# Aikku93/ulc-codec

Hardware: AMD Instinct MI355X
Metric: encode+decode Msamples/s at BlockSize=2048 stereo (channel-samples through encode+decode, VBR -50, 32 blocks per stream per call) (higher is better)
Workload: dtype f32; 1 GPU; vbr50 (configs[1] encode, configs[2] decode): Batch=4096 independent 44.1 kHz stereo streams/GPU x 32 blocks, BlockSize=2048, VBR -50; step = encode then decode; config=vbr50, mode=both, streams_per_gpu=4096, block_size=2048, channels=2, parallelism=batch split over 1 GPU(s), no collective on the data path

## Files before the change

### ulc-codec_amd/csrc/ulcx_api.cpp

```cpp
#include <math.h>
#include <stddef.h>
#include <stdio.h>
#include <stdlib.h>
#include <string.h>
#include <vector>
#include "ulcx_internal.h"


#define CKR(x) do { hipError_t e_ = (x); if (e_ != hipSuccess) { ulcx_set_error("%s: %s", #x, hipGetErrorString(e_)); return ULCX_ERR_HIP; } } while (0)

struct Block1Graph {
    hipStream_t stream = nullptr; hipGraph_t graph = nullptr; hipGraphExec_t exec = nullptr;
    bool graphed = false, noGraph = false;
};
static void block1_drop(Block1Graph &g) { if (g.graphed) { hipGraphExecDestroy(g.exec); hipGraphDestroy(g.graph); g.graphed = false; } }
template <class F> static int block1_run(Block1Graph &g, F enqueue) {
    if (!g.graphed && !g.noGraph) {
        bool ok = hipStreamBeginCapture(g.stream, hipStreamCaptureModeThreadLocal) == hipSuccess;
        if (ok) {
            const int rc = enqueue();
            hipGraph_t gr = nullptr;
            const hipError_t ee = hipStreamEndCapture(g.stream, &gr);
            ok = (rc == ULCX_OK) && ee == hipSuccess && gr != nullptr;
            if (ok) ok = hipGraphInstantiate(&g.exec, gr, nullptr, nullptr, 0) == hipSuccess;
// ... 112 lines not shown
    for (void *p : e->allocs) hipFree(p);
    if (e->tables) hipFree(e->tables);
    if (e->evOk) for (auto &v : e->ev) hipEventDestroy(v);
    block1_drop(e->b1);
    if (e->b1.stream) hipStreamDestroy(e->b1.stream);
    if (e->pinIn) hipHostFree(e->pinIn);
    if (e->pinOut) hipHostFree(e->pinOut);
    if (e->pinMeta) hipHostFree(e->pinMeta);
    enc_sync_destroy(e->sync);
    delete e;
}

static int enc_reset_state(ulcx_encoder *e) {
    UlcxEncCtx &c = e->ctx;
    CKR(hipMemset(c.hist, 0, sizeof(float) * (size_t)e->B * 2 * e->BS * e->C));
    std::vector<UlcxWcState> w((size_t)e->B);
    for (auto &x : w) {
        memset(&x, 0, sizeof(x));
        x.wcPrev = 0x10;
        x.wcCur  = 0x10;
    }
    CKR(hipMemcpy(c.wcs, w.data(), sizeof(UlcxWcState) * w.size(), hipMemcpyHostToDevice));
    return ULCX_OK;
}

extern "C" int ulcx_encoder_create(ulcx_encoder **out, int device, int nStreams, int nChan, int BlockSize, int RateHz, int maxBlocksPerCall) {
    if (!out) return ULCX_ERR_ARG;
    *out = nullptr;
    if (!validate(nChan, BlockSize) || nStreams < 1 || maxBlocksPerCall < 1 || RateHz < 1) {
        ulcx_set_error("invalid encoder geometry (nStreams=%d nChan=%d BlockSize=%d RateHz=%d maxBlocks=%d)", nStreams, nChan, BlockSize, RateHz, maxBlocksPerCall);
        return ULCX_ERR_ARG;
    }
    if (BlockSize > ULCX_MAX_BS_DEVICE) { ulcx_set_error("BlockSize %d > %d not built for the device yet", BlockSize, ULCX_MAX_BS_DEVICE); return ULCX_ERR_UNSUPPORTED; }
    int rc = select_device(device);
    if (rc) return rc;
    ulcx_encoder *e = new ulcx_encoder();
    e->device = device; e->B = nStreams; e->C = nChan; e->BS = BlockSize; e->rate = RateHz; e->maxK = maxBlocksPerCall;
    UlcxEncCtx &c = e->ctx;
    c.B = nStreams; c.C = nChan; c.BS = BlockSize; c.lgBS = ilog2i(BlockSize); c.maxK = maxBlocksPerCall; c.K = 0;
    c.rateHz = RateHz;
    c.slot = 2 * nChan * BlockSize + 16;
    c.unitCap = 2 * BlockSize + 32;
    c.cHP  = 1.0f - expf(-0x1.CC845Cp6f / RateHz);
    c.cBP  = 1.0f - expf(-0x1.596344p8f / RateHz);
    c.qHP  = 1.0f - expf(-0x1.CC845Cp7f / RateHz);
    c.qBP  = 1.0f - expf(-0x1.596344p8f / RateHz);
    c.cBlk = 1.0f - expf(-0x1.1AF110p-6f * BlockSize / RateHz);
    c.cplxScale = 0x1.62E430p-1f * (31 - __builtin_clz((unsigned)BlockSize));
    rc = ulcx_tables_build(&c.T, &e->tables, BlockSize, RateHz, true);
    if (rc) { cleanup(e); return rc; }
    {
        int most = 0;
        const int N = BlockSize / 2;
        for (int t = 0; t < 2; t++) {
            const short *beg = t ? c.T.pBeg[0] : c.T.nBeg[0], *end = t ? c.T.pEnd[0] : c.T.nEnd[0];
            for (int b = 0; b < ULCX_NBARK; b++) {
                if (beg[b] > end[b] || end[b] > N) most = 1 << 20;
                if (b && (beg[b] < beg[b - 1] || end[b] < end[b - 1])) most = 1 << 20;
            }
            for (int pos = 0; pos <= N; pos++) {
                int open = 0;
                for (int b = 0; b < ULCX_NBARK; b++) open += (beg[b] <= pos && pos <= end[b]) ? 1 : 0;
                if (open > most) most = open;
            }
        }
        int ring = 4;
        while (ring < most) ring *= 2;
        c.barkRing = (ring <= 8 && N % 32 == 0) ? ring : 0;
    }
    size_t B = nStreams, K = maxBlocksPerCall, NB = B * K, cb = (size_t)nChan * BlockSize;
    DA(c.hist, B * 2 * BlockSize * nChan, true);
    DA(c.wcs, B, true);
    DA(c.env, ((B + 63) / 64) * 64 * K * BlockSize, true);
    DA(c.bins, B * (K + 1) * 16, true);
    DA(c.wcArr, B * (K + 2), true);
    DA(c.coef, NB * cb, false);
    DA(c.key, NB * cb, false);
    DA(c.nsum, ((NB * nChan + 63) / 64) * 64 * (size_t)(BlockSize / 2), false);
    DA(c.amp2, ((NB + 63) / 64) * 64 * (size_t)(BlockSize / 2), false);
    DA(c.barkN, NB * nChan * 4 * ULCX_NBARK, true);
    DA(c.barkP, NB * 4 * ULCX_NBARK, true);
    if (c.barkRing) { DA(c.barkRawN, NB * nChan * ULCX_NBARK * 3, false); DA(c.barkRawP, NB * ULCX_NBARK * 3, false); DA(c.decList, NB, false); DA(c.decCount, 1, true); }
    DA(c.nnz, NB, true);
    DA(c.cplx, NB, true);
    DA(c.nout, NB, true);
    DA(c.slow, 3 * NB + 2, true);
    c.useWave = 1;
    c.useGapSums = (cb <= 16384 && nChan <= 16) ? 1 : 0;
    DA(c.gapSum, NB * cb, false);
    DA(c.tailSum, NB * nChan * 4 * 8, true);
    c.directPack = 1;
    if (const char *ev = getenv("ULCX_DIRECT_PACK")) c.directPack = (ev[0] != '0');
    c.dbgSkip = 0;
#ifdef ULCX_ABLATE
    if (const char *ev = getenv("ULCX_DBG_SKIP")) c.dbgSkip = atoi(ev);
#endif
    DA(c.cbrLo, NB, true); DA(c.cbrHi, NB, true); DA(c.cbrDone, NB, true); DA(c.cbrBudget, NB, true); DA(c.cbrLive, 1, true);
    DA(c.selWin, NB, true); DA(c.selT, NB, true); c.selPass = 0;
    { const char *ev = getenv("ULCX_SEL_PAIR"); c.selPair = ev ? atoi(ev) : 1; }
    DA(c.keep, NB * cb / 32, true);
    DA(c.fbList, NB, true);
    DA(c.fbCount, 4, true);
    DA(c.unitBuf, NB * nChan * (size_t)c.unitCap, true);
    DA(c.unitNyb, NB * nChan * 4, true);
    {
        size_t heapBytes = (cb * 8 > ULCX_HEAP_LDS_BYTES) ? (size_t)ULCX_HEAP_GRID * cb * 8 : 16;
        uint8_t *hp = nullptr;
        DA(hp, heapBytes, false);
        c.heapScratch = hp;
    }
    for (auto &v : e->ev) { if (hipEventCreate(&v) != hipSuccess) { ulcx_set_error("hipEventCreate failed"); cleanup(e); return ULCX_ERR_HIP; } }
    e->evOk = true;
    {
        const char *evs = getenv("ULCX_ASYNC_FB");
        const bool sideOk = !(evs && evs[0] == '0') && enc_sync_create(e->sync);
        e->wcPipe = sideOk ? 4 : 1;
        if (const char *pv = getenv("ULCX_WC_PIPE")) { int n = atoi(pv); if (n >= 1 && n <= ULCX_XF_MAXCH && n != 2 && (n == 1 || sideOk)) e->wcPipe = n; }
        if (const char *sv = getenv("ULCX_WC_STEPS")) e->wcSteps = atoi(sv);
    }
    if (const char *av = getenv("ULCX_ANALYSE_KXF")) e->analyseKxf = (av[0] == '1');
    e->nsSlots = c.useGapSums ? ulcx_enc_nsums_slots(BlockSize, nChan) : 0;
    if (e->nsSlots <= 0) e->nsSlots = 1024;
    DA(c.isFb, NB, true);
    DA(c.ownSlot, NB, true);
    {
        size_t slots = NB;
        size_t maxSlots = ((size_t)8 << 30) / (cb * 4);
        size_t freeB = 0, totalB = 0;
        if (hipMemGetInfo(&freeB, &totalB) == hipSuccess && freeB / 4 / (cb * 4) < maxSlots) maxSlots = freeB / 4 / (cb * 4);
        if (maxSlots < 64) maxSlots = 64;
        if (slots > maxSlots) slots = maxSlots;
        if (const char *ev = getenv("ULCX_RANK_SLOTS")) { long n = atol(ev); if (n >= 1 && (size_t)n < slots) slots = (size_t)n; }
        for (;;) {
            int rc_ = dalloc(e->allocs, &c.rankBuf, slots * cb, false);
            if (rc_ == ULCX_OK) break;
            if (rc_ != ULCX_ERR_NOMEM || slots <= 64) { cleanup(e); return rc_; }
            (void)hipGetLastError();
            slots = (slots + 1) / 2; if (slots < 64) slots = 64;
        }
        c.rankSlots = (int)slots;
    }
    rc = enc_reset_state(e);
    if (rc) { cleanup(e); return rc; }
    *out = e;
    return ULCX_OK;
}

extern "C" void ulcx_encoder_destroy(ulcx_encoder *e) { if (e) { hipSetDevice(e->device); cleanup(e); } }
extern "C" int ulcx_encoder_reset(ulcx_encoder *e) { if (!e) return ULCX_ERR_ARG; CKR(hipSetDevice(e->device)); return enc_reset_state(e); }
extern "C" int ulcx_encoder_slot_bytes(const ulcx_encoder *e) { return e ? e->ctx.slot : 0; }

static UlcxEncAux enc_aux(ulcx_encoder *e, int nBlocks) {
    const int wcPipe = (nBlocks >= 2 * e->wcPipe) ? e->wcPipe : (nBlocks >= 6 && e->wcPipe > 1 ? 3 : 1);
    return UlcxEncAux{ e->sync, wcPipe, e->wcSteps, e->wcFuse, e->nsSlots, e->nXf };
}

static int encode_dev_any(ulcx_encoder *e, int mode, float p0, float p1, const ulcx_rate *d_rate, const float *d_pcm, const int16_t *d_pcm16, int nBlocks,
                          uint8_t *d_out, int32_t *d_bits, int32_t *d_wc, float *d_cplx, void *hipStream) {
    if (!e || (!d_pcm && !d_pcm16) || !d_out || !d_bits || nBlocks < 1 || nBlocks > e->maxK) { ulcx_set_error("ulcx_encode_dev: bad argument"); return ULCX_ERR_ARG; }
    if (d_rate) { mode = ULCX_MODE_VBR; p0 = 100.0f; p1 = 0.0f; }
    if (mode != ULCX_MODE_VBR && mode != ULCX_MODE_CBR && mode != ULCX_MODE_ABR) { ulcx_set_error("bad mode"); return ULCX_ERR_ARG; }
    CKR(hipSetDevice(e->device));
    UlcxEncCtx c = e->ctx;
    c.K = nBlocks; c.keyFinal = 0; c.mode = mode; c.p0 = p0; c.p1 = p1;
    c.vbrTarget = (mode == ULCX_MODE_VBR) ? 0x1.E4EFB7p3f * logf(100.0f / p0) : 0.0f;
    c.rates = (const float2 *)d_rate;
// ... 533 lines not shown
extern "C" int ulcx_ulc_rate_kbps(uint64_t totalBytes, uint32_t RateHz, uint32_t BlockSize, uint32_t nBlocks) {
    double avg = (double)totalBytes * 8.0 * RateHz / 1000.0 / ((double)BlockSize * nBlocks);
    return (int)lrint(avg);
}
extern "C" int ulcx_pack_streams_dev(int device, int nStreams, int nBlocks, int slotBytes, const uint8_t *d_slots, const int32_t *d_bits,
                                     uint8_t *d_payload, long long payloadStride, int32_t *d_payloadBytes, int32_t *d_maxBlock, void *hipStream) {
    if (nStreams < 1 || nBlocks < 1 || slotBytes < 1 || !d_slots || !d_bits || !d_payload || !d_payloadBytes || payloadStride < 1) { ulcx_set_error("ulcx_pack_streams_dev: bad argument"); return ULCX_ERR_ARG; }
    int rc = select_device(device);
    if (rc) return rc;
    return ulcx_pack_launch(nStreams, nBlocks, slotBytes, d_slots, d_bits, d_payload, payloadStride, d_payloadBytes, d_maxBlock, (hipStream_t)hipStream);
}
extern "C" int ulcx_decode_packed_dev(ulcx_decoder *e, const uint8_t *d_payload, long long payloadStride, const int32_t *d_payloadBytes,
                                      int nBlocks, float *d_pcm, int32_t *d_bits, void *hipStream) {
    if (!e || !d_payload || !d_payloadBytes || !d_pcm || !d_bits || payloadStride < 1 || nBlocks < 1 || nBlocks > e->maxK) { ulcx_set_error("ulcx_decode_packed_dev: bad argument"); return ULCX_ERR_ARG; }
    CKR(hipSetDevice(e->device));
    UlcxDecCtx c = e->ctx;
    c.K = nBlocks; c.slot = 0; c.in = d_payload; c.pcm = d_pcm; c.pcm16 = nullptr; c.bits = d_bits;
    c.packed = 1; c.payStride = payloadStride; c.payBytes = d_payloadBytes;
    c.inBytes = (long long)e->B * payloadStride;
    int rc = dec_launch(e, c, (hipStream_t)hipStream);
    e->evRecorded = (rc == ULCX_OK) && e->timing;
    return rc;
}
extern "C" int ulcx_decode_packed_host(ulcx_decoder *e, const uint8_t *h_payload, long long payloadStride, const int32_t *h_payloadBytes,
                                       int nBlocks, float *h_pcm, int32_t *h_bits) {
    if (!e || !h_payload || !h_payloadBytes || !h_pcm || !h_bits || nBlocks < 1 || nBlocks > e->maxK || payloadStride < 1) return ULCX_ERR_ARG;
    CKR(hipSetDevice(e->device));
    size_t cb = (size_t)e->C * e->BS, NB = (size_t)e->B * nBlocks;
    uint8_t *dp = nullptr; int32_t *dn = nullptr; float *dpcm = nullptr; int32_t *dbits = nullptr;
    size_t payBytes = (size_t)e->B * (size_t)payloadStride + 16;
    CKR(hipMalloc((void **)&dp, payBytes)); CKR(hipMalloc((void **)&dn, sizeof(int32_t) * e->B));
    CKR(hipMalloc((void **)&dpcm, sizeof(float) * NB * cb)); CKR(hipMalloc((void **)&dbits, sizeof(int32_t) * NB));
    CKR(hipMemset(dp, 0, payBytes));
    CKR(hipMemcpy(dp, h_payload, (size_t)e->B * (size_t)payloadStride, hipMemcpyHostToDevice));
    CKR(hipMemcpy(dn, h_payloadBytes, sizeof(int32_t) * e->B, hipMemcpyHostToDevice));
    int rc = ulcx_decode_packed_dev(e, dp, payloadStride, dn, nBlocks, dpcm, dbits, nullptr);
    if (rc == ULCX_OK) {
        CKR(hipDeviceSynchronize());
        CKR(hipMemcpy(h_pcm, dpcm, sizeof(float) * NB * cb, hipMemcpyDeviceToHost));
        CKR(hipMemcpy(h_bits, dbits, sizeof(int32_t) * NB, hipMemcpyDeviceToHost));
    }
    hipFree(dp); hipFree(dn); hipFree(dpcm); hipFree(dbits);
    return rc;
}

extern "C" int ulcx_decoder_upload_payload(ulcx_decoder *e, const uint8_t *h_payload, long long payloadStride, const int32_t *h_payloadBytes) {
    if (!e || !h_payload || !h_payloadBytes || payloadStride < 1) return ULCX_ERR_ARG;
    CKR(hipSetDevice(e->device));
    if (e->d_pay) { hipFree(e->d_pay); e->d_pay = nullptr; }
    if (e->d_payBytes) { hipFree(e->d_payBytes); e->d_payBytes = nullptr; }
    size_t bytes = (size_t)e->B * (size_t)payloadStride;
    CKR(hipMalloc((void **)&e->d_pay, bytes + 16)); CKR(hipMalloc((void **)&e->d_payBytes, sizeof(int32_t) * e->B));
    CKR(hipMemset(e->d_pay, 0, bytes + 16));
    CKR(hipMemcpy(e->d_pay, h_payload, bytes, hipMemcpyHostToDevice));
    CKR(hipMemcpy(e->d_payBytes, h_payloadBytes, sizeof(int32_t) * e->B, hipMemcpyHostToDevice));
    e->payStride = payloadStride;
    return ulcx_decoder_reset(e);
}
extern "C" int ulcx_decode_resident_host(ulcx_decoder *e, int nBlocks, float *h_pcm, int32_t *h_bits) {
    if (!e || !h_pcm || !h_bits || nBlocks < 1 || nBlocks > e->maxK) return ULCX_ERR_ARG;
    if (!e->d_pay) { ulcx_set_error("ulcx_decode_resident_host: no payload uploaded"); return ULCX_ERR_ARG; }
    CKR(hipSetDevice(e->device));
    size_t cb = (size_t)e->C * e->BS, NB = (size_t)e->B * nBlocks;
    { int rc0 = dec_host_staging(e, (size_t)e->B * e->maxK, 0); if (rc0) return rc0; }
    int rc = ulcx_decode_packed_dev(e, e->d_pay, e->payStride, e->d_payBytes, nBlocks, e->d_pcm, e->d_bits, nullptr);
    if (rc != ULCX_OK) return rc;
    CKR(hipDeviceSynchronize());
    CKR(hipMemcpy(h_pcm, e->d_pcm, sizeof(float) * NB * cb, hipMemcpyDeviceToHost));
    CKR(hipMemcpy(h_bits, e->d_bits, sizeof(int32_t) * NB, hipMemcpyDeviceToHost));
    return ULCX_OK;
}

#ifdef ULCX_DSYN_STAMPS
extern "C" int ulcx_decoder_debug_scratch(ulcx_decoder *e, void *h_out, size_t strideBytes, size_t nBytes, int nStreams);
extern "C" int ulcx_decoder_debug_scratch(ulcx_decoder *e, void *h_out, size_t strideBytes, size_t nBytes, int nStreams) {
    if (!e || !h_out) return ULCX_ERR_ARG;
    CKR(hipSetDevice(e->device));
    CKR(hipDeviceSynchronize());
    for (int s = 0; s < nStreams && s < e->B; s++)
        CKR(hipMemcpy((char *)h_out + (size_t)s * nBytes, (const char *)e->ctx.scratch + (size_t)s * strideBytes, nBytes, hipMemcpyDeviceToHost));
    return ULCX_OK;
}
#endif
extern "C" int ulcx_encoder_set_timing(ulcx_encoder *e, int on) { if (!e) return ULCX_ERR_ARG; e->timing = on != 0; if (!on) e->evRecorded = false; return ULCX_OK; }
extern "C" int ulcx_decoder_set_timing(ulcx_decoder *e, int on) { if (!e) return ULCX_ERR_ARG; e->timing = on != 0; if (!on) e->evRecorded = false; return ULCX_OK; }
static const char *kDecStage[ULCX_DEC_STAGES] = { "k_dscan", "k_dsyn" };
extern "C" const char *ulcx_decoder_stage_name(int i) { return (i >= 0 && i < ULCX_DEC_STAGES) ? kDecStage[i] : ""; }
extern "C" int ulcx_decoder_stage_ms(ulcx_decoder *e, float *ms, int maxStages) {
    if (!e || !e->evRecorded) return 0;
    int n = 0;
    for (int i = 0; i < ULCX_DEC_STAGES && i < maxStages; i++) {
        float t = 0;
        if (hipEventElapsedTime(&t, e->ev[i], e->ev[i + 1]) != hipSuccess) break;
        ms[n++] = t;
    }
    return n;
}
```

### ulc-codec_amd/csrc/ulcx_enc_xf.hip

```cpp
#include "ulcx_enc_dev.h"

__device__ __forceinline__ int first_overlap(int wc, int BS) {
    unsigned p = ulcx_pattern(wc);
    int ov = BS >> (p & 7);
    if (p & 8) ov >>= (wc & 7);
    return ov;
}

__device__ __forceinline__ float win_apply(float x, int i, int S, int aL, int ovL, int aR, int ov,
                                           const float *__restrict__ rise, const float *__restrict__ fall) {
    if (i < S) return (i < aL) ? 0.0f : (i < aL + ovL) ? x * rise[i - aL] : x;
    int n = i - S;
    return (n < aR) ? x : (n < aR + ov) ? x * fall[n - aR] : 0.0f;
}

template <typename IN, int BSC, bool AN = false>
__device__ __forceinline__ int xf_fast(const UlcxEncCtx &c, float *lds, int s, int k, int blk, int tid) {
    constexpr int BS = BSC, S = BSC, M = BSC / 2, PS = 4, Mp = FFT_PADDEDS(M, PS);
    constexpr int LGM = BSC == 4096 ? 11 : 10;
    static_assert(BSC == 2048 || BSC == 4096, "sizes with a compile-time transform");
    static_assert(WG == 256 && (M / 2) % (2 * WG) == 0, "whole fold / epilogue trips per thread");
    float2 *z = (float2 *)lds;
    float2 *twl = (float2 *)(lds + (AN ? 2 : 4) * FFT_PADDEDS(BS, PS));
    float2 *zc0 = z, *zs0 = z + Mp, *zc1 = z + (AN ? 1 : 2) * Mp, *zs1 = z + 3 * Mp;
// ... 70 lines not shown
#pragma unroll
                    for (int p = 0; p < 2; p++) {
                        const int slot = p ? (1 - u) : u;
                        re[q][p][2 * slot] = mdct[2*p] * norm; re[q][p][2 * slot + 1] = mdct[2*p+1] * norm;
                    }
                }
            }
            const int j1 = kA, j2 = M - 1 - kB;
#pragma unroll
            for (int q = 0; q < 2; q++) {
                stnt((float4 *)(coefO + q * BS + 2 * j1), make_float4(re[q][0][0], re[q][0][1], re[q][0][2], re[q][0][3]));
                stnt((float4 *)(coefO + q * BS + 2 * j2), make_float4(re[q][1][0], re[q][1][1], re[q][1][2], re[q][1][3]));
            }
        }
        return 0;
    }
#pragma unroll
    for (int e0 = 0; e0 < M / 2; e0 += 2 * WG) {
        const int kA = e0 + 2 * tid, kB = e0 + 2 * tid + 1;
        const int kk2[2] = { kA, kB };
        float re[2][2][4];
        float ns[2][2][2];
        float am[2][2] = { { 0.0f, 0.0f }, { 0.0f, 0.0f } };
#pragma unroll
        for (int u = 0; u < 2; u++) {
            const int k1 = kk2[u], k2 = M - 1 - k1;
            const int r1 = (int)(__brev((unsigned)k1) >> (32 - LGM)), r2 = (int)(__brev((unsigned)k2) >> (32 - LGM));
            const float2 P1 = pre[k1], P2 = pre[k2];
            const fft_v2f Pv1 = { P1.x, P1.y }, Pv2 = { P2.x, P2.y };
#pragma unroll
            for (int q = 0; q < 2; q++) {
                const float2 *zc = q ? zc1 : zc0, *zs = q ? zs1 : zs0;
                auto cm = [](float2 d, fft_v2f w) { const fft_v2f dv = { d.x, d.y }; const fft_v2f r = fft_cmulc_post_pk(dv, w); return make_float2(r.x, r.y); };
                const float2 yc1 = cm(zc[FFT_PADS(r1, PS)], Pv1), yc2 = cm(zc[FFT_PADS(r2, PS)], Pv2);
                const float2 ys1 = cm(zs[FFT_PADS(r1, PS)], Pv1), ys2 = cm(zs[FFT_PADS(r2, PS)], Pv2);
                const float mdct[4] = { yc1.x, yc2.y, yc2.x, yc1.y };
                const float mdst[4] = { ys1.x, ys2.y, ys2.x, ys1.y };
#pragma unroll
                for (int p = 0; p < 2; p++) {
                    const float re0 = mdct[2*p] * norm,   im0 = mdst[2*p] * norm;
                    const float re1 = mdct[2*p+1] * norm, im1 = mdst[2*p+1] * norm;
                    const float re0s = re0 * re0, im0s = im0 * im0, re1s = re1 * re1, im1s = im1 * im1;
                    const float a0 = re0s + im0s, a1 = re1s + im1s;
                    nnz += (fabsf(re0) < 0.5f * ULCX_COEF_EPS) ? 0 : 1;
                    nnz += (fabsf(re1) < 0.5f * ULCX_COEF_EPS) ? 0 : 1;
                    const int slot = p ? (1 - u) : u;
                    re[q][p][2 * slot] = re0; re[q][p][2 * slot + 1] = re1;
                    ns[q][p][slot] = a0 + a1;
                    am[p][slot] += a0; am[p][slot] += a1;
                }
            }
        }
        const int j1 = kA, j2 = M - 1 - kB;
#pragma unroll
        for (int q = 0; q < 2; q++) {
            stnt((float4 *)(coefO + q * BS + 2 * j1), make_float4(re[q][0][0], re[q][0][1], re[q][0][2], re[q][0][3]));
            stnt((float4 *)(coefO + q * BS + 2 * j2), make_float4(re[q][1][0], re[q][1][1], re[q][1][2], re[q][1][3]));
            stnt((float2 *)(c.nsum + tile_idx(BS / 2, blk * 2 + q, j1)), make_float2(ns[q][0][0], ns[q][0][1]));
            stnt((float2 *)(c.nsum + tile_idx(BS / 2, blk * 2 + q, j2)), make_float2(ns[q][1][0], ns[q][1][1]));
        }
        *(float2 *)(c.amp2 + tile_idx(BS / 2, blk, j1)) = make_float2(am[0][0], am[0][1]);
        *(float2 *)(c.amp2 + tile_idx(BS / 2, blk, j2)) = make_float2(am[1][0], am[1][1]);
    }
    return nnz;
}

template <typename IN>
__device__ __forceinline__ bool xf_is_fast(const UlcxEncCtx &c, int s, int k) {
#ifdef XF_NO_FAST
    return false;
#endif
    const int BS = c.BS;
    const int *wrow = c.wcArr + (size_t)s * (c.maxK + 2) + k;
    const int wcPrev = wrow[0], wc = wrow[1], wcNext = wrow[2];
    if (!(k >= 2 || std::is_same<IN, float>::value) || (ulcx_pattern(wc) >> 4) != 0) return false;
    unsigned pp = ulcx_pattern(wcPrev);
    int lastS = BS;
    do { lastS = BS >> (pp & 7); } while (pp >>= 4);
    int ovFirst = first_overlap(wc, BS);
    if (ovFirst > lastS) ovFirst = lastS;
    return ovFirst == BS && first_overlap(wcNext, BS) >= BS;
}

template <bool ST, typename IN, bool AN = false>
__device__ __forceinline__ void xf_block(const UlcxEncCtx &c, float *lds, int s, int k, const int tid) {
    const int BS = c.BS, C = ST ? 2 : c.C;
    const int blk = s * c.K + k;
    const int ps = ulcx_xf_pad_shift(BS, C);
    float2 *z    = (float2 *)lds;
    constexpr int NA = AN ? 2 : 4;
    float2 *twl  = (float2 *)(lds + NA * FFT_PADDEDS(BS, ps));
    int    &s_nnz = *(int *)(lds + NA * FFT_PADDEDS(BS, ps) + BS / 2);
    const bool ampLds = !AN && (C > 2);
    const bool twInLds = !(ampLds && (size_t)16 * (BS + (BS >> ps)) + (size_t)BS * 4 + 32 > ULCX_LDS_LIMIT);
    float  *amp2 = twInLds ? lds + 4 * FFT_PADDEDS(BS, ps) + BS / 2 + 4 : lds + 4 * FFT_PADDEDS(BS, ps);
    if (!AN && tid == 0) s_nnz = 0;
    if (ampLds) for (int i = tid; i < BS / 2; i += WG) amp2[i] = 0.0f;

    const int *wrow = c.wcArr + (size_t)s * (c.maxK + 2) + k;
    int wcPrev = wrow[0], wc = wrow[1], wcNext = wrow[2];
    if (!AN && c.barkRing && tid == 0 && (ulcx_pattern(wc) & ~8u) != 0) c.decList[atomicAdd(c.decCount, 1)] = blk;
    int nextOv = first_overlap(wcNext, BS);
    int ovFirst;
    {
        unsigned pp = ulcx_pattern(wcPrev);
        int lastS = BS;
        do { lastS = BS >> (pp & 7); } while (pp >>= 4);
        ovFirst = first_overlap(wc, BS);
        if (ovFirst > lastS) ovFirst = lastS;
    }
    size_t cb = (size_t)C * BS;
    float *coefO = c.coef + (size_t)blk * cb;
    int nnz = 0;
    __syncthreads();

#ifdef XF_NO_FAST
    const bool fastBlk = false;
#else
    const bool fastBlk = ST && (BS == 2048 || BS == 4096) && (k >= 2 || std::is_same<IN, float>::value) && (ulcx_pattern(wc) >> 4) == 0
                         && ovFirst == BS && nextOv >= BS;
#endif
    if (fastBlk) nnz = (BS == 2048) ? xf_fast<IN, 2048, AN>(c, lds, s, k, blk, tid) : xf_fast<IN, 4096, AN>(c, lds, s, k, blk, tid);
    else
    for (int ch0 = 0; ch0 < C; ch0 += 2) {
        const int nch = ST ? 2 : ((ch0 + 1 < C) ? 2 : 1);
        unsigned pat = ulcx_pattern(wc);
        int off = 0, ovL = ovFirst;
        do {
            int S = BS >> (pat & 7);
            int d = pat & 7;
            pat >>= 4;
            int ov;
            if (pat) { ov = BS >> (pat & 7); if (pat & 8) ov >>= (wc & 7); }
            else ov = nextOv;
            if (ov > S) ov = S;
            const int M = S >> 1;
            int t0 = (k - 1) * BS - BS / 2 + off - S / 2;
            int aL = (S - ovL) >> 1, aR = (S - ov) >> 1;
            const float *rise = c.T.winRise + ovL, *fall = c.T.winFall + ov;
            const float2 *pre = c.T.pre[d];
            const int Mp = FFT_PADDEDS(M, ps);
            float2 *zc0 = z, *zs0 = z + Mp, *zc1 = z + (AN ? 1 : 2) * Mp, *zs1 = z + 3 * Mp;

            if (twInLds) for (int i = tid; i < M / 2; i += WG) twl[i] = c.T.tw[d][i];
            auto fold = [&](auto inpcmT, auto fullovT) {
                constexpr bool INPCM = decltype(inpcmT)::value, FULLOV = decltype(fullovT)::value;
                const IN *frame = pcm_base<IN>(c) + ((size_t)s * c.K * BS + (INPCM ? t0 : 0)) * C;
                auto ldE = [&](int pos, int e) -> float { return INPCM ? ld1(frame + (size_t)pos * C + e) : smp_ld1<IN>(c, s, t0 + pos, e); };
                auto ldQ = [&](int pos) -> float4 { return INPCM ? ld4(frame + (size_t)pos * C) : smp_ld4<IN>(c, s, t0 + pos); };
                for (int jj = tid; jj < M / 2; jj += WG) {
                    const int iA = 2 * jj, iB = S - 2 - 2 * jj, iC = S + 2 * jj, iD = 2 * S - 2 - 2 * jj;
                    float2 xs[8];
                    {
                        const int ip[4] = { iA, iB, iC, iD };
#pragma unroll
                        for (int r = 0; r < 4; r++) {
                            float2 e0, e1;
                            if (nch == 2) {
                                if (C == 2) { float4 v = ldQ(ip[r]); e0 = make_float2(v.x, v.y); e1 = make_float2(v.z, v.w); }
                                else { e0 = make_float2(ldE(ip[r], ch0), ldE(ip[r], ch0 + 1)); e1 = make_float2(ldE(ip[r] + 1, ch0), ldE(ip[r] + 1, ch0 + 1)); }
                                xs[2 * r]     = make_float2((e0.x + e0.y) * 0.5f, (e0.x - e0.y) * 0.5f);
                                xs[2 * r + 1] = make_float2((e1.x + e1.y) * 0.5f, (e1.x - e1.y) * 0.5f);
                            } else {
                                xs[2 * r] = make_float2(ldE(ip[r], ch0), 0.0f); xs[2 * r + 1] = make_float2(ldE(ip[r] + 1, ch0), 0.0f);
                            }
                        }
                    }
                    const int ipos[8] = { iA, iA + 1, iB, iB + 1, iC, iC + 1, iD, iD + 1 };
#pragma unroll
                    for (int r = 0; r < 8; r++) {
                        if (FULLOV) {
                            float f = (r < 4) ? rise[ipos[r]] : fall[ipos[r] - S];
                            xs[r].x *= f; xs[r].y *= f;
                            continue;
                        }
                        float f; bool zero;
                        if (r < 4) {
                            int idx = ipos[r] - aL;
                            int ci = idx < 0 ? 0 : (idx < ovL ? idx : 0);
                            float tv = rise[ci];
                            f = (idx < ovL) ? tv : 1.0f; zero = idx < 0;
                        } else {
                            int idx = ipos[r] - S - aR;
                            int ci = idx < 0 ? 0 : (idx < ov ? idx : 0);
                            float tv = fall[ci];
                            f = (idx < 0) ? 1.0f : tv; zero = idx >= ov;
                        }
                        float wx = xs[r].x * f, wy = xs[r].y * f;
                        xs[r].x = zero ? 0.0f : wx;
                        xs[r].y = zero ? 0.0f : wy;
                    }
#pragma unroll
                    for (int hsel = 0; hsel < 2; hsel++) {
                        const int n = hsel ? M / 2 + jj : M / 2 - 1 - jj;
                        const float2 lbv = hsel ? xs[0] : xs[1], lav = hsel ? xs[3] : xs[2];
                        const float2 rav = hsel ? xs[4] : xs[5], rbv = hsel ? xs[7] : xs[6];
                        float2 P = pre[n];
#pragma unroll
                        for (int q = 0; q < 2; q++) {
                            if (q >= nch) break;
                            float ra = q ? rav.y : rav.x, rb = q ? rbv.y : rbv.x, la = q ? lav.y : lav.x, lb = q ? lbv.y : lbv.x;
                            float vr = ra + rb, wr = ra - rb;
                            float vl = la - lb, wl = lb + la;
                            float v1 = hsel ? vl : vr, v2 = hsel ? vr : vl;
                            float w1 = hsel ? wl : wr, w2 = hsel ? wr : wl;
                            float2 *zc = q ? zc1 : zc0, *zs = q ? zs1 : zs0;
                            zc[FFT_PADS(n, ps)] = cmulc(make_float2(v1, v2), P);
                            if constexpr (!AN) zs[FFT_PADS(n, ps)] = cmulc(make_float2(w2, w1), P);
                        }
                    }
                }
            };
            if (!(ULCX_DBG(c) & 2)) {
                const bool inPcm = (t0 >= 0), fullOv = (ovL == S) && (ov == S);
                if (inPcm && fullOv) fold(std::true_type{}, std::true_type{});
                else if (inPcm) fold(std::true_type{}, std::false_type{});
                else fold(std::false_type{}, std::false_type{});
            }
            __syncthreads();

            if (!(ULCX_DBG(c) & 1)) for (int a = __builtin_amdgcn_readfirstlane(tid >> 6); a < (AN ? 1 : 2) * nch; a += WG / 64) {
                if (twInLds) fft_wave_dif(z + a * Mp, M, twl, tid & 63, ps);
                else fft_wave_dif(z + a * Mp, M, c.T.tw[d], tid & 63, ps);
            }
            __syncthreads();

            int bits = 31 - __clz(M);
            float norm = 2.0f / S;
            if (!(ULCX_DBG(c) & 4)) for (int kk = tid; kk < M / 2; kk += WG) {
                int k1 = kk, k2 = M - 1 - kk;
                int r1 = (int)(__brev((unsigned)k1) >> (32 - bits));
                int r2 = (int)(__brev((unsigned)k2) >> (32 - bits));
                float2 P1 = pre[k1], P2 = pre[k2];
                float am1 = 0.0f, am2 = 0.0f;
                if (ampLds) { am1 = amp2[off / 2 + k1]; am2 = amp2[off / 2 + k2]; }
#pragma unroll
                for (int q = 0; q < 2; q++) {
                    if (q >= nch) break;
                    int ch = ch0 + q;
                    float2 *zc = q ? zc1 : zc0, *zs = q ? zs1 : zs0;
                    const fft_v2f Pv1 = { P1.x, P1.y }, Pv2 = { P2.x, P2.y };
                    auto cm = [](float2 d, fft_v2f w) { const fft_v2f dv = { d.x, d.y }; const fft_v2f r = fft_cmulc_post_pk(dv, w); return make_float2(r.x, r.y); };
                    float2 yc1 = cm(zc[FFT_PADS(r1, ps)], Pv1), yc2 = cm(zc[FFT_PADS(r2, ps)], Pv2);
                    if constexpr (AN) {
                        const float mdctA[4] = { yc1.x, yc2.y, yc2.x, yc1.y };
#pragma unroll
                        for (int p = 0; p < 2; p++) {
                            const int j = p ? k2 : k1;
                            stnt((float2 *)(coefO + (size_t)ch * BS + off + 2 * j), make_float2(mdctA[2*p] * norm, mdctA[2*p+1] * norm));
                        }
                        continue;
                    }
                    float2 ys1 = cm(zs[FFT_PADS(r1, ps)], Pv1), ys2 = cm(zs[FFT_PADS(r2, ps)], Pv2);
                    float mdct[4] = { yc1.x, yc2.y, yc2.x, yc1.y };
                    float mdst[4] = { ys1.x, ys2.y, ys2.x, ys1.y };
#pragma unroll
                    for (int p = 0; p < 2; p++) {
                        float re0 = mdct[2*p] * norm,   im0 = mdst[2*p] * norm;
                        float re1 = mdct[2*p+1] * norm, im1 = mdst[2*p+1] * norm;
                        float re0s = re0 * re0, im0s = im0 * im0, re1s = re1 * re1, im1s = im1 * im1;
                        float a0 = re0s + im0s, a1 = re1s + im1s;
                        nnz += (fabsf(re0) < 0.5f * ULCX_COEF_EPS) ? 0 : 1;
                        nnz += (fabsf(re1) < 0.5f * ULCX_COEF_EPS) ? 0 : 1;
                        int j = p ? k2 : k1;
                        size_t gi = (size_t)ch * BS + off + 2 * j;
                        stnt((float2 *)(coefO + gi), make_float2(re0, re1));
                        stnt(c.nsum + tile_idx(BS / 2, blk * C + ch, off / 2 + j), a0 + a1);
                        if (p) { am2 += a0; am2 += a1; } else { am1 += a0; am1 += a1; }
                    }
                }
                if (AN) continue;
                if (ampLds) { amp2[off / 2 + k1] = am1; amp2[off / 2 + k2] = am2; }
                else { c.amp2[tile_idx(BS / 2, blk, off / 2 + k1)] = am1; c.amp2[tile_idx(BS / 2, blk, off / 2 + k2)] = am2; }
            }
            __syncthreads();
            off += S; ovL = ov;
        } while (pat);
    }
    if (AN) return;
    for (int o = 32; o > 0; o >>= 1) nnz += __shfl_down(nnz, o);
    if ((tid & 63) == 0) atomicAdd(&s_nnz, nnz);
    if (ampLds) for (int i = tid; i < BS / 2; i += WG) c.amp2[tile_idx(BS / 2, blk, i)] = amp2[i];
    __syncthreads();
    if (tid == 0) c.nnz[blk] = s_nnz;
}

#ifndef ULCX_XF_ANALYSIS_UNIT
template <bool ST, typename IN>
__global__ __launch_bounds__(WG, 4) void k_xf(UlcxEncCtx c, int k0, int k1) {
    extern __shared__ float lds[];
    const int kc = k1 - k0;
    const int NBk = c.B * kc;
    const int per = (NBk + 7) / 8;
    const int vb = (int)(blockIdx.x % 8) * per + (int)(blockIdx.x / 8);
    if (vb >= NBk) return;
    xf_block<ST, IN>(c, lds, vb / kc, k0 + vb % kc, threadIdx.x);
}
#else
template <bool ST, typename IN>
__global__ __launch_bounds__(WG, XFA_LB) void k_xfa(UlcxEncCtx c, int k0, int k1) {
    extern __shared__ float lds[];
    const int kc = k1 - k0;
    const int NBk = c.B * kc;
    const int per = (NBk + 7) / 8;
    const int vb = (int)(blockIdx.x % 8) * per + (int)(blockIdx.x / 8);
    if (vb >= NBk) return;
    xf_block<ST, IN, true>(c, lds, vb / kc, k0 + vb % kc, threadIdx.x);
}
#endif

template <typename IN, bool AN>
__device__ __forceinline__ void xf_big_block(const UlcxEncCtx &c, int k0, int k1) {
    extern __shared__ float lds[];
    const int BS = c.BS, C = c.C;
    const int kc = k1 - k0;
    const int NBk = c.B * kc;
    const int vb = blockIdx.x;
    if (vb >= NBk) return;
    const int s = vb / kc, k = k0 + vb % kc;
    const int blk = s * c.K + k;
    const int tid = threadIdx.x;
    float2 *z = (float2 *)lds;
    __shared__ int s_nnz;
    if (tid == 0) s_nnz = 0;
    const int *wrow = c.wcArr + (size_t)s * (c.maxK + 2) + k;
    const int wcPrev = wrow[0], wc = wrow[1], wcNext = wrow[2];
    if (!AN && c.barkRing && threadIdx.x == 0 && (ulcx_pattern(wc) & ~8u) != 0) c.decList[atomicAdd(c.decCount, 1)] = blk;
    const int nextOv = first_overlap(wcNext, BS);
    int ovFirst;
    {
        unsigned pp = ulcx_pattern(wcPrev);
        int lastS = BS;
        do { lastS = BS >> (pp & 7); } while (pp >>= 4);
        ovFirst = first_overlap(wc, BS);
        if (ovFirst > lastS) ovFirst = lastS;
    }
    const size_t cb = (size_t)C * BS;
    float *coefO = c.coef + (size_t)blk * cb;
    int nnz = 0;
    __syncthreads();
    for (int ch = 0; ch < C; ch++) {
        unsigned pat = ulcx_pattern(wc);
        int off = 0, ovL = ovFirst;
        do {
            const int S = BS >> (pat & 7);
            const int d = pat & 7;
            pat >>= 4;
            int ov;
            if (pat) { ov = BS >> (pat & 7); if (pat & 8) ov >>= (wc & 7); }
            else ov = nextOv;
            if (ov > S) ov = S;
            const int M = S >> 1;
            const int t0 = (k - 1) * BS - BS / 2 + off - S / 2;
            const int aL = (S - ovL) >> 1, aR = (S - ov) >> 1;
            const float *rise = c.T.winRise + ovL, *fall = c.T.winFall + ov;
            const float2 *pre = c.T.pre[d];
            const int bits = 31 - __clz(M);
            const float norm = 2.0f / S;
            for (int kind = 0; kind < (AN ? 1 : 2); kind++) {
                for (int jj = tid; jj < M / 2; jj += WG) {
                    const int iA = 2 * jj, iB = S - 2 - 2 * jj, iC = S + 2 * jj, iD = 2 * S - 2 - 2 * jj;
                    const int ipos[8] = { iA, iA + 1, iB, iB + 1, iC, iC + 1, iD, iD + 1 };
                    float xs[8];
#pragma unroll
                    for (int r = 0; r < 8; r++) xs[r] = win_apply(ms_sample<IN>(c, s, t0 + ipos[r], ch), ipos[r], S, aL, ovL, aR, ov, rise, fall);
#pragma unroll
                    for (int hsel = 0; hsel < 2; hsel++) {
// ... 233 lines not shown
```

### ulc-codec_amd/csrc/ulcx_internal.h

```cpp
#pragma once
#include <hip/hip_runtime.h>
#include <stdint.h>
#include "../../include/ulc_amd.h"

#ifndef ULCX_DSYN_TWL
#define ULCX_DSYN_TWL 1
#endif
#define ULCX_NBARK 25
#define ULCX_MAX_SUB 4
#define ULCX_BARK_EVENTS 52
#define ULCX_MAX_BS_DEVICE 32768
#define ULCX_COEF_EPS (0x1.0p-31f)
#define ULCX_HEAP_LDS_BYTES (128 * 1024)
#define ULCX_HEAP_GRID 256
#define ULCX_DONE_VBR 2
#ifdef ULCX_ABLATE
#define ULCX_DBG(c) ((c).dbgSkip)
#else
#define ULCX_DBG(c) 0
#endif

struct UlcxTables {
    const float2 *pre[ULCX_MAX_SUB];
    const float2 *tw[ULCX_MAX_SUB];
    const float  *winFall;
    const float  *winRise;
    const int    *bandIdx[ULCX_MAX_SUB];
    const float  *bandFrac[ULCX_MAX_SUB];
    const float4 *bandW[ULCX_MAX_SUB];
    const uint32_t *barkSched;
    short nBeg[ULCX_MAX_SUB][ULCX_NBARK], nEnd[ULCX_MAX_SUB][ULCX_NBARK];
    short pBeg[ULCX_MAX_SUB][ULCX_NBARK], pEnd[ULCX_MAX_SUB][ULCX_NBARK];
};

struct UlcxWcState {
    float tf[3];
    int   wcPrev, wcCur;
    float binSum[8], binW[8];
    int   pad;
};

struct UlcxEncCtx {
    int B, K, C, BS, lgBS;
    int barkRing;
    int *decList, *decCount;
    int maxK;
    int slot;
    int unitCap;
    int mode; float p0, p1;
    float vbrTarget;
    const float2 *rates;
    float cHP, cBP, qHP, qBP, cBlk;
    float cplxScale;
    int   rateHz;
    UlcxTables T;
    int keyFinal;
    const float *pcm; const int16_t *pcm16;
    uint8_t *out; int32_t *bits; int32_t *wcOut; float *cplxOut;
    float *hist;
    UlcxWcState *wcs;
    float2 *env;
    float  *bins;
    int    *wcArr;
    float  *coef;
    float  *key;
    float  *nsum;
    float  *npair;
    float  *amp2;
    float  *barkN;
    float  *barkP;
    double *barkRawN, *barkRawP;
    int    *nnz;
    float  *cplx;
    int    *nout;
    int    *cbrLo, *cbrHi, *cbrDone;
    uint32_t *keep;
    int    *fbList; int *fbCount;
    uint8_t *unitBuf;
    int    *unitNyb;
    int    *cbrBudget;
    uint4  *selWin;
    uint32_t *selT;
    int     selPair;
    int     selPass;
    int    *cbrLive;
    int    *slow;
    float2 *gapSum;
    float  *tailSum;
    int     useGapSums;
    int    *isFb;
    int    *ownSlot;
    int    *rankBuf;
    int     dbgSkip;
    int     forceFb;
    int     rankSlots, fbLo, fbHi;
    int     fbMode;
    int     useWave;
    int     directPack;
    void   *heapScratch;
};

struct UlcxDecCtx {
    int B, K, C, BS, lgBS, maxK;
    int s0, s1;
    int slot;
    int dbgSkip;
    UlcxTables T;
    const uint8_t *in; float *pcm; int16_t *pcm16;
    long long inBytes;
    int32_t *bits;
    float *lap;
    int   *lastSub;
    uint32_t *seed;
    int   *dead;
    float *lapO; int *lastSubO; uint32_t *seedO; int *deadO;
    float *lapScratch;
    int    synFull;
    int    k0, k1;
    int   *wcScan;
    int   *draws;
    int   *unitDraws;
    float4 *unitTail;
    int4  *unitRec;
    uint2 *prec; int precStride;
    uint2 *nrec; int nrecStride;
    float *tailMag;
    int    tailStride;
    float *scratch;
    const uint32_t *jumpT;
    const uint32_t *parT;
    int    fastOK, twInLds;
    int   packed;
    long long payStride;
    const int32_t *payBytes;
    int  *packOff;
    int  *blkOff;
};

__host__ __device__ static inline unsigned ulcx_pattern(int wc) {
    const unsigned i = ((unsigned)wc >> 4) & 15u;
    const unsigned long long t0 = 0x0091001900080000ull, t1 = 0x0A2102A101A2012Aull, t2 = 0x1B3213B212B3123Bull, t3 = 0xB3213B212B3123B1ull;
    const unsigned long long t = (i & 8u) ? ((i & 4u) ? t3 : t2) : ((i & 4u) ? t1 : t0);
    return (unsigned)(t >> (16u * (i & 3u))) & 0xFFFFu;
}

int  ulcx_tables_build(UlcxTables *devT, void **devBlob, int BS, int rateHz, bool forEncoder);
void ulcx_set_error(const char *fmt, ...);

#define ULCX_ENC_STAGES 20
#define ULCX_ENC_STAGES_REPORTED (ULCX_ENC_STAGES + 1)
extern const char *const ulcx_enc_stage_names[ULCX_ENC_STAGES_REPORTED];
#define ULCX_DEC_STAGES 2
#define ULCX_WC_MAXCH 32
#define ULCX_XF_MAXCH 8
#define ULCX_LDS_LIMIT (160 * 1024)
struct UlcxEncSync {
    hipEvent_t wcStart, wcForward[ULCX_WC_MAXCH], wcBackward[ULCX_WC_MAXCH], wcDecided[ULCX_WC_MAXCH];
    hipEvent_t xfChunkDone[ULCX_XF_MAXCH], cplxChunksDone;
    hipEvent_t noiseFork, noiseDone, tailFork, tailDone;
    hipEvent_t cplxDone, stateDone;
    hipEvent_t exactFork, exactFork2, exactJoin;
    hipEvent_t xfTiming[2 * ULCX_XF_MAXCH];
    hipStream_t side, side2, side3;
};
struct UlcxEncAux {
    UlcxEncSync &sync;
    int wcPipe;
    int wcSteps, wcFuse, nsSlots;
    int &nXf;
};
int ulcx_enc_launch(const UlcxEncCtx &c, hipStream_t st, hipEvent_t *ev , const UlcxEncAux &aux);
struct UlcxDecAux {
    int synGrid;
    int synFull;
};
int ulcx_dec_launch(const UlcxDecCtx &c, hipStream_t st, hipEvent_t *ev, const UlcxDecAux &aux);
size_t ulcx_dec_lds_bytes(int BS, int C, int fast, int twInLds);
int ulcx_dec_syn_slots(const UlcxDecCtx &c);
int ulcx_pack_launch(int nStreams, int nBlocks, int slotBytes, const uint8_t *d_slots, const int32_t *d_bits, uint8_t *d_payload,
                     long long stride, int32_t *d_payloadBytes, int32_t *d_maxBlock, hipStream_t st);
int ulcx_analyse_launch(const UlcxEncCtx &c, hipStream_t st, hipEvent_t *ev, const UlcxEncAux &aux, int useKxf);
int ulcx_enc_nsums_slots(int BS, int C);
// ... 9 lines not shown
```

Before: 55550 Msamples/s.

## Add dedicated stereo transform path for blocks split into subblocks

Adds a specialized xf_subblocks routine for stereo blocks whose window pattern splits them into several transient subblocks. It folds all subblocks together, runs one wave-level FFT per subblock, and writes the coefficient, noise-sum and amplitude outputs in a single pass instead of taking the generic per-channel-pair path. It also adds optional per-block timing stamps behind a compile flag. This adds code complexity and shared-memory layout assumptions for the subblock case, and only helps when transient blocks are common.

```diff
diff --git a/ulc-codec_amd/csrc/ulcx_api.cpp b/ulc-codec_amd/csrc/ulcx_api.cpp
--- a/ulc-codec_amd/csrc/ulcx_api.cpp
+++ b/ulc-codec_amd/csrc/ulcx_api.cpp
@@ -218,6 +218,9 @@
     DA(c.barkP, NB * 4 * ULCX_NBARK, true);
     if (c.barkRing) { DA(c.barkRawN, NB * nChan * ULCX_NBARK * 3, false); DA(c.barkRawP, NB * ULCX_NBARK * 3, false); DA(c.decList, NB, false); DA(c.decCount, 1, true); }
     DA(c.nnz, NB, true);
+#ifdef ULCX_XF_STAMPS
+    DA(c.xfStamps, NB, true);
+#endif
     DA(c.cplx, NB, true);
     DA(c.nout, NB, true);
     DA(c.slow, 3 * NB + 2, true);
@@ -917,6 +920,16 @@
     return ULCX_OK;
 }
 #endif
+#ifdef ULCX_XF_STAMPS
+extern "C" int ulcx_encoder_debug_xf_stamps(ulcx_encoder *e, int nBlocks, unsigned long long *h_out);
+extern "C" int ulcx_encoder_debug_xf_stamps(ulcx_encoder *e, int nBlocks, unsigned long long *h_out) {
+    if (!e || !h_out || nBlocks < 1 || nBlocks > e->maxK) return ULCX_ERR_ARG;
+    CKR(hipSetDevice(e->device));
+    CKR(hipDeviceSynchronize());
+    CKR(hipMemcpy(h_out, e->ctx.xfStamps, sizeof(unsigned long long) * (size_t)e->B * nBlocks, hipMemcpyDeviceToHost));
+    return ULCX_OK;
+}
+#endif
 extern "C" int ulcx_encoder_set_timing(ulcx_encoder *e, int on) { if (!e) return ULCX_ERR_ARG; e->timing = on != 0; if (!on) e->evRecorded = false; return ULCX_OK; }
 extern "C" int ulcx_decoder_set_timing(ulcx_decoder *e, int on) { if (!e) return ULCX_ERR_ARG; e->timing = on != 0; if (!on) e->evRecorded = false; return ULCX_OK; }
 static const char *kDecStage[ULCX_DEC_STAGES] = { "k_dscan", "k_dsyn" };
diff --git a/ulc-codec_amd/csrc/ulcx_enc_xf.hip b/ulc-codec_amd/csrc/ulcx_enc_xf.hip
--- a/ulc-codec_amd/csrc/ulcx_enc_xf.hip
+++ b/ulc-codec_amd/csrc/ulcx_enc_xf.hip
@@ -176,8 +176,170 @@
     return ovFirst == BS && first_overlap(wcNext, BS) >= BS;
 }
 
+template <typename IN, bool AN>
+__device__ __forceinline__ int xf_subblocks(const UlcxEncCtx &c, float *lds, int s, int k, int blk, const int tid, int wc, int ovFirst, int nextOv) {
+    const int BS = c.BS, ps = ulcx_xf_pad_shift(BS, 2);
+    constexpr int NA = AN ? 2 : 4;
+    float2 *z = (float2 *)lds, *twl = (float2 *)(lds + NA * FFT_PADDEDS(BS, ps));
+    const unsigned pat0 = ulcx_pattern(wc);
+    auto each = [&](auto f) {
+        unsigned pat = pat0;
+        int off = 0, ovL = ovFirst;
+        do {
+            const int d = pat & 7, S = BS >> d;
+            pat >>= 4;
+            int ov;
+            if (pat) { ov = BS >> (pat & 7); if (pat & 8) ov >>= (wc & 7); }
+            else ov = nextOv;
+            if (ov > S) ov = S;
+            f(off, d, S, ovL, ov);
+            off += S; ovL = ov;
+        } while (pat);
+    };
+    auto twoff = [&](int d) { return d ? (BS >> 2) - (BS >> (d + 1)) : 0; };
+    struct Sub { int off, S, ovL, ov; const float2 *pre; };
+    auto pick = [&](int i) {
+        Sub m = { 0, 0, 0, 0, nullptr };
+        each([&](int off, int d, int S, int ovL, int ov) { if (4 * i >= off) { m.off = off; m.S = S; m.ovL = ovL; m.ov = ov; m.pre = c.T.pre[d]; } });
+        return m;
+    };
+    {
+        unsigned seen = 0;
+        each([&](int, int d, int S, int, int) {
+            if (!((seen >> d) & 1u)) { const float2 *tw = c.T.tw[d]; float2 *dst = twl + twoff(d); for (int i = tid; i < (S >> 2); i += WG) dst[i] = tw[i]; }
+            seen |= 1u << d;
+        });
+    }
+    auto fold = [&](auto inpcmT) {
+        constexpr bool INPCM = decltype(inpcmT)::value;
+        const IN *pcmS = pcm_base<IN>(c) + (size_t)s * c.K * BS * 2;
+        for (int fi = tid; fi < (BS >> 2); fi += WG) {
+            const Sub m = pick(fi);
+            const int S = m.S, M = S >> 1, jj = fi - (m.off >> 2), ovL = m.ovL, ov = m.ov;
+            const int t0 = (k - 1) * BS - BS / 2 + m.off - S / 2;
+            const int aL = (S - ovL) >> 1, aR = (S - ov) >> 1;
+            const float *rise = c.T.winRise + ovL, *fall = c.T.winFall + ov;
+            const float2 *pre = m.pre;
+            const int Mp = FFT_PADDEDS(M, ps);
+            float2 *zc0 = z + NA * FFT_PADS(m.off >> 1, ps), *zs0 = zc0 + Mp, *zc1 = zc0 + (AN ? 1 : 2) * Mp, *zs1 = zc0 + 3 * Mp;
+            const int iA = 2 * jj, iB = S - 2 - 2 * jj, iC = S + 2 * jj, iD = 2 * S - 2 - 2 * jj;
+            const int ip[4] = { iA, iB, iC, iD };
+            float4 v[4];
+#pragma unroll
+            for (int r = 0; r < 4; r++) v[r] = INPCM ? ld4(pcmS + (size_t)(t0 + ip[r]) * 2) : smp_ld4<IN>(c, s, t0 + ip[r]);
+            float2 xs[8];
+#pragma unroll
+            for (int r = 0; r < 4; r++) {
+                xs[2 * r]     = make_float2((v[r].x + v[r].y) * 0.5f, (v[r].x - v[r].y) * 0.5f);
+                xs[2 * r + 1] = make_float2((v[r].z + v[r].w) * 0.5f, (v[r].z - v[r].w) * 0.5f);
+            }
+            const int ipos[8] = { iA, iA + 1, iB, iB + 1, iC, iC + 1, iD, iD + 1 };
+#pragma unroll
+            for (int r = 0; r < 8; r++) {
+                float f; bool zero;
+                if (r < 4) {
+                    int idx = ipos[r] - aL;
+                    int ci = idx < 0 ? 0 : (idx < ovL ? idx : 0);
+                    float tv = rise[ci];
+                    f = (idx < ovL) ? tv : 1.0f; zero = idx < 0;
+                } else {
+                    int idx = ipos[r] - S - aR;
+                    int ci = idx < 0 ? 0 : (idx < ov ? idx : 0);
+                    float tv = fall[ci];
+                    f = (idx < 0) ? 1.0f : tv; zero = idx >= ov;
+                }
+                float wx = xs[r].x * f, wy = xs[r].y * f;
+                xs[r].x = zero ? 0.0f : wx;
+                xs[r].y = zero ? 0.0f : wy;
+            }
+#pragma unroll
+            for (int hsel = 0; hsel < 2; hsel++) {
+                const int n = hsel ? M / 2 + jj : M / 2 - 1 - jj;
+                const float2 lbv = hsel ? xs[0] : xs[1], lav = hsel ? xs[3] : xs[2];
+                const float2 rav = hsel ? xs[4] : xs[5], rbv = hsel ? xs[7] : xs[6];
+                const float2 P = pre[n];
+#pragma unroll
+                for (int q = 0; q < 2; q++) {
+                    const float ra = q ? rav.y : rav.x, rb = q ? rbv.y : rbv.x, la = q ? lav.y : lav.x, lb = q ? lbv.y : lbv.x;
+                    const float vr = ra + rb, wr = ra - rb;
+                    const float vl = la - lb, wl = lb + la;
+                    const float v1 = hsel ? vl : vr, v2 = hsel ? vr : vl;
+                    const float w1 = hsel ? wl : wr, w2 = hsel ? wr : wl;
+                    float2 *zc = q ? zc1 : zc0, *zs = q ? zs1 : zs0;
+                    zc[FFT_PADS(n, ps)] = cmulc(make_float2(v1, v2), P);
+                    if constexpr (!AN) zs[FFT_PADS(n, ps)] = cmulc(make_float2(w2, w1), P);
+                }
+            }
+        }
+    };
+    if (k >= 2) fold(std::true_type{}); else fold(std::false_type{});
+    __syncthreads();
+
+    {
+        const int a = __builtin_amdgcn_readfirstlane(tid >> 6);
+        if (a < NA) each([&](int off, int d, int S, int, int) {
+            const int M = S >> 1;
+            fft_wave_dif(z + NA * FFT_PADS(off >> 1, ps) + a * FFT_PADDEDS(M, ps), M, twl + twoff(d), tid & 63, ps);
+        });
+    }
+    __syncthreads();
+
+    float *coefO = c.coef + (size_t)blk * (2 * BS);
+    int nnz = 0;
+    for (int ei = tid; ei < (BS >> 2); ei += WG) {
+        const Sub m = pick(ei);
+        const int S = m.S, M = S >> 1, off = m.off, kk = ei - (off >> 2);
+        const float2 *pre = m.pre;
+        const int Mp = FFT_PADDEDS(M, ps);
+        const float2 *zc0 = z + NA * FFT_PADS(off >> 1, ps), *zs0 = zc0 + Mp, *zc1 = zc0 + (AN ? 1 : 2) * Mp, *zs1 = zc0 + 3 * Mp;
+        const int bits = 31 - __clz(M);
+        const float norm = 2.0f / S;
+        const int k1 = kk, k2 = M - 1 - kk;
+        const int r1 = (int)(__brev((unsigned)k1) >> (32 - bits));
+        const int r2 = (int)(__brev((unsigned)k2) >> (32 - bits));
+        const float2 P1 = pre[k1], P2 = pre[k2];
+        const fft_v2f Pv1 = { P1.x, P1.y }, Pv2 = { P2.x, P2.y };
+        float am1 = 0.0f, am2 = 0.0f;
+#pragma unroll
+        for (int q = 0; q < 2; q++) {
+            const float2 *zc = q ? zc1 : zc0, *zs = q ? zs1 : zs0;
+            auto cm = [](float2 d, fft_v2f w) { const fft_v2f dv = { d.x, d.y }; const fft_v2f r = fft_cmulc_post_pk(dv, w); return make_float2(r.x, r.y); };
+            const float2 yc1 = cm(zc[FFT_PADS(r1, ps)], Pv1), yc2 = cm(zc[FFT_PADS(r2, ps)], Pv2);
+            const float mdct[4] = { yc1.x, yc2.y, yc2.x, yc1.y };
+            if constexpr (AN) {
+#pragma unroll
+                for (int p = 0; p < 2; p++) {
+                    const int j = p ? k2 : k1;
+                    stnt((float2 *)(coefO + (size_t)q * BS + off + 2 * j), make_float2(mdct[2*p] * norm, mdct[2*p+1] * norm));
+                }
+            } else {
+                const float2 ys1 = cm(zs[FFT_PADS(r1, ps)], Pv1), ys2 = cm(zs[FFT_PADS(r2, ps)], Pv2);
+                const float mdst[4] = { ys1.x, ys2.y, ys2.x, ys1.y };
+#pragma unroll
+                for (int p = 0; p < 2; p++) {
+                    const float re0 = mdct[2*p] * norm,   im0 = mdst[2*p] * norm;
+                    const float re1 = mdct[2*p+1] * norm, im1 = mdst[2*p+1] * norm;
+                    const float re0s = re0 * re0, im0s = im0 * im0, re1s = re1 * re1, im1s = im1 * im1;
+                    const float a0 = re0s + im0s, a1 = re1s + im1s;
+                    nnz += (fabsf(re0) < 0.5f * ULCX_COEF_EPS) ? 0 : 1;
+                    nnz += (fabsf(re1) < 0.5f * ULCX_COEF_EPS) ? 0 : 1;
+                    const int j = p ? k2 : k1;
+                    stnt((float2 *)(coefO + (size_t)q * BS + off + 2 * j), make_float2(re0, re1));
+                    stnt(c.nsum + tile_idx(BS / 2, blk * 2 + q, off / 2 + j), a0 + a1);
+                    if (p) { am2 += a0; am2 += a1; } else { am1 += a0; am1 += a1; }
+                }
+            }
+        }
+        if constexpr (!AN) { c.amp2[tile_idx(BS / 2, blk, off / 2 + k1)] = am1; c.amp2[tile_idx(BS / 2, blk, off / 2 + k2)] = am2; }
+    }
+    return nnz;
+}
+
 template <bool ST, typename IN, bool AN = false>
 __device__ __forceinline__ void xf_block(const UlcxEncCtx &c, float *lds, int s, int k, const int tid) {
+#ifdef ULCX_XF_STAMPS
+    const unsigned long long stamp0 = __builtin_amdgcn_s_memtime();
+#endif
     const int BS = c.BS, C = ST ? 2 : c.C;
     const int blk = s * c.K + k;
     const int ps = ulcx_xf_pad_shift(BS, C);
@@ -214,7 +376,13 @@
     const bool fastBlk = ST && (BS == 2048 || BS == 4096) && (k >= 2 || std::is_same<IN, float>::value) && (ulcx_pattern(wc) >> 4) == 0
                          && ovFirst == BS && nextOv >= BS;
 #endif
+#ifdef XF_NO_SUBBLOCKS
+    const bool subBlk = false;
+#else
+    const bool subBlk = ST && BS <= 4096 && (ulcx_pattern(wc) >> 4) != 0;
+#endif
     if (fastBlk) nnz = (BS == 2048) ? xf_fast<IN, 2048, AN>(c, lds, s, k, blk, tid) : xf_fast<IN, 4096, AN>(c, lds, s, k, blk, tid);
+    else if (subBlk) { if constexpr (ST) nnz = xf_subblocks<IN, AN>(c, lds, s, k, blk, tid, wc, ovFirst, nextOv); }
     else
     for (int ch0 = 0; ch0 < C; ch0 += 2) {
         const int nch = ST ? 2 : ((ch0 + 1 < C) ? 2 : 1);
@@ -377,6 +545,12 @@
     if (ampLds) for (int i = tid; i < BS / 2; i += WG) c.amp2[tile_idx(BS / 2, blk, i)] = amp2[i];
     __syncthreads();
     if (tid == 0) c.nnz[blk] = s_nnz;
+#ifdef ULCX_XF_STAMPS
+    if (tid == 0) {
+        const unsigned cls = fastBlk ? 0u : (ulcx_pattern(wc) >> 4) != 0 ? 2u : (ovFirst != BS || nextOv < BS) ? 1u : 3u;
+        c.xfStamps[blk] = ((__builtin_amdgcn_s_memtime() - stamp0) << 2) | cls;
+    }
+#endif
 }
 
 #ifndef ULCX_XF_ANALYSIS_UNIT
diff --git a/ulc-codec_amd/csrc/ulcx_internal.h b/ulc-codec_amd/csrc/ulcx_internal.h
--- a/ulc-codec_amd/csrc/ulcx_internal.h
+++ b/ulc-codec_amd/csrc/ulcx_internal.h
@@ -98,6 +98,9 @@
     int     useWave;
     int     directPack;
     void   *heapScratch;
+#ifdef ULCX_XF_STAMPS
+    unsigned long long *xfStamps;
+#endif
 };
 
 struct UlcxDecCtx {
```

Result: no change. 55540 Msamples/s (-0.0%).
